# keya-dialog/LoCo-ASR

Hardware: AMD Instinct MI355X
Metric: audio frames/sec SpeechT5-base encoder, 30s×bs32 @1/2/4/8 GPU; embed L2 vs HF (higher is better)
Workload: dtype f16x3 (fp16 hi+lo operands, 3 MFMAs per product, fp32 accumulate); 1 GPU; SpeechT5-base speech encoder, synthetic 16 kHz 30 s clips, batch 32 per GPU (BASELINE.json configs[1]), random-init weights; batch_per_gpu=32, global_batch=32, frames_per_clip=1499, parallelism=dp1, collective=none

## Files before the change

### loco-asr_amd/csrc/attention_f16x3.hip

```cpp
#include <cstdlib>

#include "loco_kernels.h"

namespace loco {

typedef _Float16 h8 __attribute__((ext_vector_type(8)));
typedef float f32x2 __attribute__((ext_vector_type(2)));
typedef unsigned u32x4 __attribute__((ext_vector_type(4)));
typedef _Float16 h4 __attribute__((ext_vector_type(4)));

constexpr int AX_BQ = 128, AX_BK = 64;
constexpr int AX_PL = AX_BK * kHeadDim;
constexpr int AX_STG = 2 * AX_PL;

typedef __attribute__((address_space(1))) const void* ax_gptr_t;
typedef __attribute__((address_space(3))) void* ax_lptr_t;

#ifndef LOCO_ATTN_HACK
#define LOCO_ATTN_HACK 0
#endif
#define AX_MFMA(a, b, c) __builtin_amdgcn_mfma_f32_32x32x16_f16(a, b, c, 0, 0, 0)
#define AX_PIN() __builtin_amdgcn_sched_barrier(0)

#ifdef LOCO_ATTN_STAMPS
__device__ unsigned long long* g_attn_stamps = nullptr;
#define AX_STAMP(k_)                                                                                                     \
    {                                                                                                                    \
        unsigned long long t_;                                                                                           \
        __builtin_amdgcn_sched_barrier(0);                                                                               \
        asm volatile("s_memtime %0\n\ts_waitcnt lgkmcnt(0)" : "=s"(t_) :: "memory");                                     \
        __builtin_amdgcn_sched_barrier(0);                                                                               \
        seg[k_] += t_ - tlast;                                                                                           \
        tlast = t_;                                                                                                      \
    }
#else
#define AX_STAMP(k_) {}
#endif

__device__ __forceinline__ void ax_split_pair(const f32x2 pv, unsigned& hi, unsigned& lo) {
    asm("s_nop 0\n\tv_cvt_pk_f16_f32 %0, %1, %2" : "=v"(hi) : "v"(pv.x), "v"(pv.y));
    asm("v_fma_mixlo_f16 %0, %1, 1.0, -%2 op_sel_hi:[0,0,1]" : "=v"(lo) : "v"(pv.x), "v"(hi));
    asm("v_fma_mixhi_f16 %0, %1, 1.0, -%2 op_sel:[0,0,1] op_sel_hi:[0,0,1]" : "+v"(lo) : "v"(pv.y), "v"(hi));
}

#ifdef LOCO_ATTN_DEBUG
__device__ float* g_attn_dbg = nullptr;
#define AX_DBG(tile_, code_, S0_, S1_)                                                                                   \
    if (g_attn_dbg && (tile_) < 8) {                                                                                     \
        float* d_ = g_attn_dbg + (((long)blockIdx.x * 256 + tid) * 8 + (tile_)) * 8;                                     \
        unsigned mask_ = 0;                                                                                              \
        float smax_ = -INFINITY, smin_ = INFINITY;                                                                       \
        _Pragma("unroll") for (int e = 0; e < 16; ++e) {                                                                 \
            if (!(fabsf(S0_[e]) <= 3e38f) && S0_[e] != -INFINITY) mask_ |= 1u;                                           \
            if (!(fabsf(S1_[e]) <= 3e38f) && S1_[e] != -INFINITY) mask_ |= 1u;                                           \
            smax_ = fmaxf(smax_, fmaxf(S0_[e], S1_[e])); smin_ = fminf(smin_, fminf(S0_[e], S1_[e]));                    \
            if (!(fabsf(o0[e]) <= 3e38f) || !(fabsf(o1[e]) <= 3e38f)) mask_ |= 2u;                                       \
        }                                                                                                                \
        if (!(fabsf(l_run) <= 3e38f)) mask_ |= 4u;                                                                       \
        if (!(fabsf(alpha) <= 3e38f)) mask_ |= 8u;                                                                       \
        if (!(fabsf(dsh) <= 3e38f)) mask_ |= 16u;                                                                        \
        d_[0] = __uint_as_float(mask_ | ((code_) << 16)); d_[1] = m_run; d_[2] = alpha; d_[3] = dsh; d_[4] = l_run;      \
        d_[5] = smax_; d_[6] = smin_; d_[7] = o0[0];                                                                     \
    }
#else
#define AX_DBG(tile_, code_, S0_, S1_) {}
#endif

typedef __fp16 ax_tr4_t __attribute__((__vector_size__(4 * sizeof(__fp16))));
__device__ __forceinline__ h8 ax_join_tr(ax_tr4_t a, ax_tr4_t b) {
    const h4 x = __builtin_bit_cast(h4, a), y = __builtin_bit_cast(h4, b);
    return h8{x[0], x[1], x[2], x[3], y[0], y[1], y[2], y[3]};
}

template <bool OUT_SPLIT, bool TABLE, bool LONG_SEQ>
__global__ __launch_bounds__(256, 2) void attention_f16x3_kernel(const _Float16* __restrict__ qhi, const _Float16* __restrict__ qlo,
                                                                 const _Float16* __restrict__ khi, const _Float16* __restrict__ klo,
                                                                 const _Float16* __restrict__ vhi, const _Float16* __restrict__ vlo,
                                                                 float* qp, const int32_t* __restrict__ frames,
                                                                 _Float16* __restrict__ ctx_hi, _Float16* __restrict__ ctx_lo,
                                                                 float* __restrict__ ctx, int T, int nqb,
                                                                 const _Float16* __restrict__ pe_hi, const _Float16* __restrict__ pe_lo,
                                                                 float pe_scale) {
    __shared__ __attribute__((aligned(16))) _Float16 lds[4 * AX_STG];
    __shared__ __attribute__((aligned(16))) float bias_stage[4][32 * 17];

    int qblk, head, b;
    {
        const int nblk = gridDim.x;
        const int q8 = nblk >> 3, r8 = nblk & 7;
        const int xcd = blockIdx.x & 7, idx = blockIdx.x >> 3;
        const int w = (xcd < r8 ? xcd * (q8 + 1) : r8 * (q8 + 1) + (xcd - r8) * q8) + idx;
        qblk = w - (w / nqb) * nqb;
        const int rest = w / nqb;
        head = rest - (rest / kHeads) * kHeads;
        b = rest / kHeads;
    }
    const int tid = threadIdx.x, lane = tid & 63;
    const int wave = __builtin_amdgcn_readfirstlane(tid >> 6);
    const int r = lane & 31, h = lane >> 5;
    const int iw0 = qblk * AX_BQ + wave * 32;
    const int iq = iw0 + r;
    const int iqc = iq < T ? iq : T - 1;

    int nvalid = frames ? frames[b] : T;
    if (nvalid <= 0 || nvalid > T) nvalid = T;
    const int ntiles = (nvalid + AX_BK - 1) / AX_BK;
    constexpr float kLog2e = 1.4426950408889634f;

    h8 qh[4], ql[4];
    {
        const long qo = ((long)b * T + iqc) * kHidden + head * kHeadDim + 8 * h;
#pragma unroll
        for (int ks = 0; ks < 4; ++ks) {
            qh[ks] = *reinterpret_cast<const h8*>(qhi + qo + 16 * ks);
            ql[ks] = *reinterpret_cast<const h8*>(qlo + qo + 16 * ks);
        }
    }
    float* qprow = qp + (((long)b * kHeads + head) * T + iqc) * kRelN;

    const int drow = lane >> 3, dpos = lane & 7;
    const unsigned lds0 = (unsigned)(unsigned long)(ax_lptr_t)lds;
    unsigned kvc[2], vvc;
#pragma unroll
    for (int i = 0; i < 2; ++i) {
        const int swz = (((2 * wave + i) & 3) << 1) | ((drow >> 1) & 1);
        kvc[i] = 2u * (unsigned)(head * kHeadDim + 8 * (dpos ^ swz));
    }
    vvc = 2u * (unsigned)(head * kHeadDim + 8 * (dpos ^ (((drow >> 1) & 1) << 2)));
    const char* const kbase_h = reinterpret_cast<const char*>(khi + (long)b * T * kHidden);
    const char* const kbase_l = reinterpret_cast<const char*>(klo + (long)b * T * kHidden);
    const char* const vbase_h = reinterpret_cast<const char*>(vhi + (long)b * T * kHidden);
    const char* const vbase_l = reinterpret_cast<const char*>(vlo + (long)b * T * kHidden);
#define AX_DMA16(base_, voff_, ldsb_) \
    asm volatile("s_mov_b32 m0, %0\n\ts_nop 0\n\tglobal_load_lds_dwordx4 %1, %2" :: "s"(ldsb_), "v"(voff_), "s"(base_) : "memory")
#define AX_DMA_PIECE(pc_, tk_, tv_, kslot_, vslot_)                                                                          \
    {                                                                                                                        \
        const int i_ = ((pc_) >> 1) & 1, pl_ = (pc_) & 1;                                                                    \
        const bool isk_ = (pc_) < 4;                                                                                         \
        const int tt_ = isk_ ? (tk_) : (tv_);                                                                                \
        const int rmax_ = T - 1 - tt_ * AX_BK;           \
        int row_ = 8 * (2 * wave + i_) + drow;                                                                               \
        row_ = row_ < rmax_ ? row_ : rmax_;                                                                                  \
        const unsigned vo_ = (unsigned)row_ * (2u * kHidden) + (isk_ ? kvc[i_] : vvc);                                       \
        const unsigned d_ = lds0 + 2u * (unsigned)((isk_ ? (kslot_) : 2 + (vslot_)) * AX_STG + pl_ * AX_PL + 8 * (2 * wave + i_) * kHeadDim); \
        AX_DMA16((isk_ ? (pl_ ? kbase_l : kbase_h) : (pl_ ? vbase_l : vbase_h)) + (long)tt_ * (AX_BK * kHidden * 2), vo_, d_); \
    }

    int fo[4];
    {
        const int swz = (((r >> 3) & 3) << 1) | ((r >> 1) & 1);
#pragma unroll
        for (int y = 0; y < 4; ++y) fo[y] = r * kHeadDim + 8 * ((2 * y + h) ^ swz);
    }
#define AX_KF(kb_, st_, ks_, pl_) (*reinterpret_cast<const h8*>((kb_) + (pl_) * AX_PL + (st_) * 32 * kHeadDim + fo[ks_]))
    int vfo[2];
    {
        const int q = (lane >> 2) & 3, pp = lane & 3, g = (lane >> 4) & 1;
#pragma unroll
        for (int dt = 0; dt < 2; ++dt)
            vfo[dt] = (4 * h + q) * kHeadDim + 8 * ((4 * (dt ^ ((q >> 1) & 1))) + 2 * g + (pp >> 1)) + 4 * (pp & 1);
    }
    typedef __fp16 ax_tr4 __attribute__((__vector_size__(4 * sizeof(__fp16))));
    typedef __attribute__((address_space(3))) ax_tr4* ax_tr4_lptr;
#define AX_VTR(vb_, dt_, c_, u_, pl_) \
    __builtin_amdgcn_ds_read_tr16_b64_v4f16((ax_tr4_lptr)((vb_) + (pl_) * AX_PL + (16 * (c_) + 8 * (u_)) * kHeadDim + vfo[dt_]))
#define AX_VF(vb_, dt_, c_, pl_) ax_join_tr(AX_VTR(vb_, dt_, c_, 0, pl_), AX_VTR(vb_, dt_, c_, 1, pl_))

    f32x16 o0, o1;
#pragma unroll
    for (int e = 0; e < 16; ++e) { o0[e] = 0.f; o1[e] = 0.f; }
    float m_run = -INFINITY, l_run = 0.f;
    float alpha = 0.f, dsh = 0.f;

    float bandv[2][2][8];
#define AX_IS_BAND(tt_) (iw0 - ((tt_) * AX_BK + AX_BK - 1) < kRelMax - 1 && iw0 + 31 - (tt_) * AX_BK > -kRelMax)
#define AX_BAND_LOAD(tt_)                                                                                              \
    if (AX_IS_BAND(tt_)) {                                                                                             \
        const float* qpb = qp + ((long)b * kHeads + head) * T * kRelN;                                                 \
        const int lj = lane & 15, lq = lane >> 4;                                                                      \
        _Pragma("unroll") for (int st_ = 0; st_ < 2; ++st_)                                                            \
            _Pragma("unroll") for (int half = 0; half < 2; ++half) {                                                   \
                const int j = (tt_) * AX_BK + 32 * st_ + 16 * half + lj;                                               \
                _Pragma("unroll") for (int u = 0; u < 8; ++u) {                                                        \
                    const int i = iw0 + 4 * u + lq;                                                                    \
                    int rel = i - j;                                                                                   \
                    rel = rel < -kRelMax ? -kRelMax : (rel > kRelMax - 1 ? kRelMax - 1 : rel);                         \
                    bandv[st_][half][u] = qpb[(long)(i < T ? i : T - 1) * kRelN + rel + kRelMax];                      \
                }                                                                                                      \
            }                                                                                                          \
    }
#define AX_BAND_ADD(S_, st_)                                                                                           \
    _Pragma("unroll") for (int half = 0; half < 2; ++half) {                                                           \
        _Pragma("unroll") for (int u = 0; u < 8; ++u) sc[66 * u + band_wr] = bandv[st_][half][u];                      \
        __builtin_amdgcn_wave_barrier();                                                                               \
        _Pragma("unroll") for (int e8 = 0; e8 < 8; ++e8)                                                               \
            S_[8 * half + e8] += sc[band_rd + (e8 & 3) + 8 * (e8 >> 2)];                                               \
        __builtin_amdgcn_wave_barrier();                                                                               \
    }
#define AX_FINISH_TILE(S0_, S1_, tt_, mx_)                                                                             \
    {                                                                                                                  \
        const int j0 = (tt_) * AX_BK;                                                                                  \
        const int dmin = iw0 - (j0 + AX_BK - 1);                                                                       \
        const int dmax = iw0 + 31 - j0;                                                                                \
        float cb = 0.f;                                                                                                \
        bool redo = false;                                                                                             \
        if (dmin >= kRelMax - 1) {                                                                                     \
            cb = c_past;                                                                                               \
        } else if (dmax <= -kRelMax) {                                                                                 \
            cb = c_future;                                                                                             \
        } else {                                                                                                       \
            float* sc = bias_stage[wave];                                                                              \
            const int lj = lane & 15, lq = lane >> 4;                                                                  \
            const int band_wr = 16 * lq + (lq >> 1) + lj, band_rd = 16 * r + (r >> 1) + 4 * h;                         \
            AX_BAND_ADD(S0_, 0)                                                                                        \
            AX_BAND_ADD(S1_, 1)                                                                                        \
            redo = true;                                                                                               \
        }                                                                                                              \
        if (j0 + AX_BK > nvalid) {                                                                                     \
            _Pragma("unroll") for (int e = 0; e < 16; ++e) {                                                           \
                const int j = j0 + (e & 3) + 8 * (e >> 2) + 4 * h;                                                     \
                S0_[e] = j < nvalid ? S0_[e] : -INFINITY;                                                              \
                S1_[e] = j + 32 < nvalid ? S1_[e] : -INFINITY;                                                         \
            }                                                                                                          \
            redo = true;                                                                                               \
        }                                                                                                              \
        float mxv = (mx_);                                                                                             \
        if (redo) {                                                                                                    \
            mxv = S0_[0];                                                                                              \
            _Pragma("unroll") for (int e = 1; e < 16; ++e) mxv = fmaxf(mxv, S0_[e]);                                   \
            _Pragma("unroll") for (int e = 0; e < 16; ++e) mxv = fmaxf(mxv, S1_[e]);                                   \
        }                                                                                                              \
        {                                               \
            float ma_ = mxv, mb_ = mxv;                                                                                \
            asm volatile("s_nop 1\n\tv_permlane32_swap_b32 %0, %1\n\ts_nop 1" : "+v"(ma_), "+v"(mb_));                \
            mxv = fmaxf(ma_, mb_) + cb;                                                                                \
        }                                                                                                              \
        const float m_new = fmaxf(m_run, mxv);                                                                         \
        alpha = __builtin_amdgcn_exp2f((m_run - m_new) * kLog2e);                                                      \
        m_run = m_new;                                                                                                 \
        dsh = (cb - m_new) * kLog2e;                                                                                   \
    }

#ifdef LOCO_ATTN_STAMPS
    unsigned long long seg[6] = {0, 0, 0, 0, 0, 0}, tlast, tstart;
    asm volatile("s_memtime %0\n\ts_waitcnt lgkmcnt(0)" : "=s"(tstart) :: "memory");
    tlast = tstart;
#endif
#pragma unroll
    for (int pc = 0; pc < 8; ++pc) AX_DMA_PIECE(pc, 0, 0, 0, 0)
    float c_past, c_future;
    if (TABLE) {
        int bmin, bmax;
        {
            int lo = iw0 - (ntiles * AX_BK - 1), hi = iw0 + 31;
            lo = lo < -kRelMax ? -kRelMax : lo;
            hi = hi > kRelMax - 1 ? kRelMax - 1 : hi;
            bmin = (lo + kRelMax) >> 5;
            bmax = (hi + kRelMax) >> 5;
        }
        float cf = 0.f, cp = 0.f;
        unsigned pev[2];
#pragma unroll
        for (int i = 0; i < 2; ++i) {
            const int swz = (((2 * wave + i) & 3) << 1) | ((drow >> 1) & 1);
            pev[i] = (unsigned)(8 * (2 * wave + i) + drow) * (2u * kHeadDim) + 16u * (unsigned)(dpos ^ swz);
        }
        const unsigned bs0 = (unsigned)(unsigned long)(ax_lptr_t)&bias_stage[0][0];
        const unsigned pev1 = (unsigned)(8 * wave + drow) * (2u * kHeadDim) + 16u * (unsigned)(dpos ^ (((wave & 3) << 1) | ((drow >> 1) & 1)));
        constexpr int kBsPlane = 32 * kHeadDim;
#define AX_PE_DMA2(b0_, slot_)                                                                                                     \
    _Pragma("unroll") for (int pc_ = 0; pc_ < 4; ++pc_) {                                                                          \
        const int i_ = (pc_ >> 1) & 1, pl_ = pc_ & 1;                                                                              \
        const unsigned d_ = lds0 + 2u * (unsigned)((slot_) * AX_STG + pl_ * AX_PL + 8 * (2 * wave + i_) * kHeadDim);               \
        AX_DMA16(reinterpret_cast<const char*>(pl_ ? pe_lo : pe_hi) + (long)(b0_) * (32 * kHeadDim * 2), pev[i_], d_);             \
    }
#define AX_PE_DMA1(b0_)                                                                                                            \
    _Pragma("unroll") for (int pl_ = 0; pl_ < 2; ++pl_) {                                                                          \
        const unsigned d_ = bs0 + 2u * (unsigned)(pl_ * kBsPlane + 8 * wave * kHeadDim);                                           \
        AX_DMA16(reinterpret_cast<const char*>(pl_ ? pe_lo : pe_hi) + (long)(b0_) * (32 * kHeadDim * 2), pev1, d_);                \
    }
        constexpr int kBlocksPerRound = kRelN / 64;
        static_assert(2 * kBlocksPerRound * 32 == kRelN && sizeof(bias_stage) >= 2 * kBsPlane * sizeof(_Float16), "table rounds");
#define AX_PE_ROUND_DMA(rd_)                                                                      \
    AX_PE_DMA2(LOCO_ATTN_HACK == 1 ? 0 : kBlocksPerRound * (rd_), 1)                               \
    AX_PE_DMA2(LOCO_ATTN_HACK == 1 ? 0 : kBlocksPerRound * (rd_) + 2, 3)                           \
    AX_PE_DMA1(LOCO_ATTN_HACK == 1 ? 0 : kBlocksPerRound * (rd_) + 4)
        AX_PE_ROUND_DMA(0)
#pragma unroll
        for (int rd = 0; rd < 2; ++rd) {
            asm volatile("s_waitcnt vmcnt(0)" ::: "memory");
            __syncthreads();
            f32x16 acc[kBlocksPerRound];
#pragma unroll
            for (int bb = 0; bb < kBlocksPerRound; ++bb) {
                const _Float16* pb = bb == 4 ? reinterpret_cast<const _Float16*>(&bias_stage[0][0]) : lds + ((bb >> 1) ? 3 : 1) * AX_STG;
                const int plane = bb == 4 ? kBsPlane : AX_PL;
#pragma unroll
                for (int e = 0; e < 16; ++e) acc[bb][e] = 0.f;
                const int blk_ = kBlocksPerRound * rd + bb;
                if (blk_ < bmin || blk_ > bmax) continue;
#pragma unroll
                for (int ks = 0; ks < 4; ++ks) {
                    const h8 fh = *reinterpret_cast<const h8*>(pb + (bb & 1) * 32 * kHeadDim + fo[ks]);
                    const h8 fl = *reinterpret_cast<const h8*>(pb + plane + (bb & 1) * 32 * kHeadDim + fo[ks]);
                    acc[bb] = AX_MFMA(fl, qh[ks], acc[bb]);
                    acc[bb] = AX_MFMA(fh, ql[ks], acc[bb]);
                    acc[bb] = AX_MFMA(fh, qh[ks], acc[bb]);
                }
            }
            __syncthreads();
            if (rd == 0) {
                AX_PE_ROUND_DMA(1)
            } else {
                const int t1 = ntiles > 1 ? 1 : 0;
#pragma unroll
                for (int pc = 0; pc < 4; ++pc) AX_DMA_PIECE(pc, t1, 0, 1, 0)
            }
#pragma unroll
            for (int bb = 0; bb < kBlocksPerRound; ++bb) {
                const int blk = kBlocksPerRound * rd + bb;
#pragma unroll
                for (int e = 0; e < 16; ++e) acc[bb][e] *= pe_scale;
                if (blk == 0) cf = acc[bb][0];
                if (blk == kRelN / 32 - 1) cp = acc[bb][15];
                if (iq < T && blk >= bmin && blk <= bmax && (LOCO_ATTN_HACK != 2 || T < 0)) {
#pragma unroll
                    for (int g4 = 0; g4 < 4; ++g4)
                        *reinterpret_cast<float4*>(qprow + 32 * blk + 8 * g4 + 4 * h) =
                            make_float4(acc[bb][4 * g4], acc[bb][4 * g4 + 1], acc[bb][4 * g4 + 2], acc[bb][4 * g4 + 3]);
                }
            }
        }
#undef AX_PE_ROUND_DMA
#undef AX_PE_DMA2
#undef AX_PE_DMA1
        float cf2 = cf, cp2 = cp;
        asm volatile("s_nop 1\n\tv_permlane32_swap_b32 %0, %1\n\ts_nop 1" : "+v"(cf), "+v"(cf2));
        asm volatile("s_nop 1\n\tv_permlane32_swap_b32 %0, %1\n\ts_nop 1" : "+v"(cp2), "+v"(cp));
        c_future = cf;
        c_past = cp;
    } else {
        const int t1 = ntiles > 1 ? 1 : 0;
#pragma unroll
        for (int pc = 0; pc < 4; ++pc) AX_DMA_PIECE(pc, t1, 0, 1, 0)
        c_past = qprow[kRelN - 1];
        c_future = qprow[0];
    }
    asm volatile("s_waitcnt vmcnt(0)" ::: "memory");
    __syncthreads();

    f32x16 sa0, sa1, sb0, sb1;
    {
#pragma unroll
        for (int e = 0; e < 16; ++e) { sa0[e] = 0.f; sa1[e] = 0.f; }
        const _Float16* kb = lds;
#pragma unroll
        for (int ks = 0; ks < 4; ++ks) {
            const h8 kh0 = AX_KF(kb, 0, ks, 0), kl0 = AX_KF(kb, 0, ks, 1), kh1 = AX_KF(kb, 1, ks, 0), kl1 = AX_KF(kb, 1, ks, 1);
            sa0 = AX_MFMA(kl0, qh[ks], sa0); sa1 = AX_MFMA(kl1, qh[ks], sa1);
            sa0 = AX_MFMA(kh0, ql[ks], sa0); sa1 = AX_MFMA(kh1, ql[ks], sa1);
            sa0 = AX_MFMA(kh0, qh[ks], sa0); sa1 = AX_MFMA(kh1, qh[ks], sa1);
        }
        float mx = sa0[0];
#pragma unroll
        for (int e = 1; e < 16; ++e) mx = fmaxf(mx, sa0[e]);
#pragma unroll
        for (int e = 0; e < 16; ++e) mx = fmaxf(mx, sa1[e]);
        AX_BAND_LOAD(0)
        AX_FINISH_TILE(sa0, sa1, 0, mx)
    }
    __syncthreads();
    AX_STAMP(5)

#define AX_ITER(t_, SC0, SC1, SN0, SN1)                                                                                \
    {                                                                                                                  \
        const int tq = (t_);                                                                                           \
        const int tkn = tq + 2 < ntiles ? tq + 2 : ntiles - 1, tvn = tq + 1 < ntiles ? tq + 1 : ntiles - 1;             \
        if (tq + 1 < ntiles) { AX_BAND_LOAD(tq + 1) }                                                                  \
        const _Float16* kb = lds + ((tq + 1) & 1) * AX_STG;                                                            \
        const _Float16* vb = lds + (2 + (tq & 1)) * AX_STG;                                                            \
        h8 kf[2][4];                                                                 \
        kf[0][0] = AX_KF(kb, 0, 0, 0); kf[0][1] = AX_KF(kb, 0, 0, 1);                                                  \
        kf[0][2] = AX_KF(kb, 1, 0, 0); kf[0][3] = AX_KF(kb, 1, 0, 1);                                                  \
        const f32x2 al2 = {alpha, alpha}, k2 = {kLog2e, kLog2e}, d2 = {dsh, dsh};                                      \
        f32x2 ps2 = {0.f, 0.f};                                                                                        \
           \
        if (!LONG_SEQ || __builtin_amdgcn_ballot_w64(alpha != 1.0f) != 0) {                                            \
            _Pragma("unroll") for (int e = 0; e < 16; e += 2) {                                                        \
                f32x2 a_ = {o0[e], o0[e + 1]}, c_ = {o1[e], o1[e + 1]};                                                \
                a_ *= al2; c_ *= al2;                                                                                  \
                o0[e] = a_.x; o0[e + 1] = a_.y; o1[e] = c_.x; o1[e + 1] = c_.y;                                        \
            }                                                                                                          \
        }                                                                                                              \
        _Pragma("unroll") for (int e = 0; e < 16; ++e) { SN0[e] = 0.f; SN1[e] = 0.f; }                                 \
        u32x4 ph0[2], pl0[2], ph1[2], pl1[2];                                                                          \
        AX_PIN();                                                                                                      \
        AX_STAMP(0)                                                                                                    \
                                                                                                     \
        _Pragma("unroll") for (int ks = 0; ks < 4; ++ks) {                                                             \
            if (ks + 1 < 4) {                                                                                          \
                kf[(ks + 1) & 1][0] = AX_KF(kb, 0, ks + 1, 0); kf[(ks + 1) & 1][1] = AX_KF(kb, 0, ks + 1, 1);          \
                kf[(ks + 1) & 1][2] = AX_KF(kb, 1, ks + 1, 0); kf[(ks + 1) & 1][3] = AX_KF(kb, 1, ks + 1, 1);          \
            }                                                                                                          \
            _Pragma("unroll") for (int m = 0; m < 6; ++m) {                                                            \
                const int st = m & 1, wh = m >> 1;                                                                     \
                const h8 a_ = kf[ks & 1][2 * st + (wh == 0 ? 1 : 0)];                                                  \
                const h8 b_ = wh == 1 ? ql[ks] : qh[ks];                                                               \
                if (st == 0) SN0 = AX_MFMA(a_, b_, SN0); else SN1 = AX_MFMA(a_, b_, SN1);                              \
                const int n = 6 * ks + m, q_ = n / 3;                                                                  \
                if (n % 3 == 0) {                                                                                      \
                    const int e0 = 2 * q_;                                                                             \
                    const f32x2 sx = {SC0[e0], SC0[e0 + 1]};                                                           \
                    const f32x2 ax = __builtin_elementwise_fma(sx, k2, d2);                                            \
                    const f32x2 pv = {__builtin_amdgcn_exp2f(ax.x), __builtin_amdgcn_exp2f(ax.y)};                     \
                    ps2 += pv;                                                                                         \
                    asm volatile("" : "+v"(ps2));                                                                      \
                    unsigned hi_, lo_;                                                                                 \
                    ax_split_pair(pv, hi_, lo_);                                                                       \
                    ph0[q_ >> 2][q_ & 3] = hi_; pl0[q_ >> 2][q_ & 3] = lo_;                                            \
                } else if (n % 3 == 1) {                                                                               \
                    const int e0 = 2 * q_;                                                                             \
                    const f32x2 sx = {SC1[e0], SC1[e0 + 1]};                                                           \
                    const f32x2 ax = __builtin_elementwise_fma(sx, k2, d2);                                            \
                    SC1[e0] = __builtin_amdgcn_exp2f(ax.x); SC1[e0 + 1] = __builtin_amdgcn_exp2f(ax.y);                \
                }                                                                                                      \
                if (n % 3 == 1 && (LOCO_ATTN_HACK != 3 || ((n / 3) & 1) == 0)) {  \
                    AX_PIN();                                                                                          \
                    AX_DMA_PIECE(n / 3, tkn, tvn, tq & 1, (tq + 1) & 1)                                                \
                }                                                                                                      \
                AX_PIN();                                                                                              \
            }                                                                                                          \
        }                                                                                                              \
        AX_STAMP(1)                                                                                                    \
                             \
        h8 vf[2][2];                                                                             \
        vf[0][0] = AX_VF(vb, 0, 0, 0); vf[0][1] = AX_VF(vb, 0, 0, 1);                                                  \
        float mxr = -INFINITY;                                                                                         \
        _Pragma("unroll") for (int g = 0; g < 8; ++g) {                                                                \
            const int st = g >> 2, s2 = (g >> 1) & 1, dt = g & 1;                                                      \
            if (g + 1 < 8) {                                                                                           \
                const int c1 = (g + 1) >> 1, dt1 = (g + 1) & 1;                                                        \
                vf[(g + 1) & 1][0] = AX_VF(vb, dt1, c1, 0); vf[(g + 1) & 1][1] = AX_VF(vb, dt1, c1, 1);                \
            }                                                                                                          \
            const h8 vh = vf[g & 1][0], vl = vf[g & 1][1];                                                             \
            const h8 ph = __builtin_bit_cast(h8, st == 0 ? ph0[s2] : ph1[s2]);                                         \
            const h8 pl = __builtin_bit_cast(h8, st == 0 ? pl0[s2] : pl1[s2]);                                         \
            _Pragma("unroll") for (int m = 0; m < 3; ++m) {                                                            \
                const h8 a_ = m == 0 ? vl : vh;                                                                        \
                const h8 b_ = m == 1 ? pl : ph;                                                                        \
                if (dt == 0) o0 = AX_MFMA(a_, b_, o0); else o1 = AX_MFMA(a_, b_, o1);                                  \
                const int n = 3 * g + m;                                                                               \
                if (n < 8) {                          \
                    const f32x2 pv = {SC1[2 * n], SC1[2 * n + 1]};                                                     \
                    ps2 += pv;                                                                                         \
                    asm volatile("" : "+v"(ps2));                                                                      \
                    unsigned hi_, lo_;                                                                                 \
                    ax_split_pair(pv, hi_, lo_);                                                                       \
                    ph1[n >> 2][n & 3] = hi_; pl1[n >> 2][n & 3] = lo_;                                                \
                } else if (n >= 12 && n < 20) {              \
                    const int e0 = 4 * (n - 12);                                                                       \
                    if (e0 < 16) mxr = fmaxf(fmaxf(fmaxf(mxr, SN0[e0]), fmaxf(SN0[e0 + 1], SN0[e0 + 2])), SN0[e0 + 3]); \
                    else mxr = fmaxf(fmaxf(fmaxf(mxr, SN1[e0 - 16]), fmaxf(SN1[e0 - 15], SN1[e0 - 14])), SN1[e0 - 13]); \
                    asm volatile("" : "+v"(mxr));                                                                      \
                }                                                                                                      \
                AX_PIN();                                                                                              \
            }                                                                                                          \
        }                                                                                                              \
        l_run = l_run * alpha + (ps2.x + ps2.y);                                                                       \
        AX_STAMP(2)                                                                                                    \
        if (tq + 1 < ntiles) { AX_FINISH_TILE(SN0, SN1, tq + 1, mxr) }                                                 \
        AX_DBG(tq, 1u, SN0, SN1)                                                                                       \
        AX_STAMP(3)                                                                                                    \
        asm volatile("s_waitcnt vmcnt(0)" ::: "memory");                                                               \
        __syncthreads();                                                                                               \
        AX_STAMP(4)                                                                                                    \
    }

    for (int t = 0; t < ntiles; t += 2) {
        AX_ITER(t, sa0, sa1, sb0, sb1)
        if (t + 1 >= ntiles) break;
        AX_ITER(t + 1, sb0, sb1, sa0, sa1)
    }
#undef AX_ITER
#undef AX_FINISH_TILE
#undef AX_BAND_LOAD
#undef AX_BAND_ADD
#undef AX_IS_BAND
#undef AX_DMA_PIECE
#undef AX_DMA16
#undef AX_KF
#undef AX_VF
#undef AX_VTR

#ifdef LOCO_ATTN_STAMPS
    if (g_attn_stamps && tid == 0) {
        unsigned long long* o_ = g_attn_stamps + 8l * blockIdx.x;
        for (int k_ = 0; k_ < 6; ++k_) o_[k_] = seg[k_];
        o_[6] = (unsigned long long)ntiles;
        o_[7] = tlast - tstart;
    }
#endif
    const float l_tot = l_run + __shfl_xor(l_run, 32, 64);
    const float inv = 1.0f / l_tot;
    if (iq < T) {
        const long obase = ((long)b * T + iq) * kHidden + head * kHeadDim + 4 * h;
#pragma unroll
        for (int g4 = 0; g4 < 4; ++g4) {
            float a[4], c[4];
#pragma unroll
            for (int e = 0; e < 4; ++e) {
                a[e] = o0[4 * g4 + e] * inv;
                c[e] = o1[4 * g4 + e] * inv;
            }
            if (OUT_SPLIT) {
                typedef unsigned u32x2 __attribute__((ext_vector_type(2)));
                unsigned h0, l0, h1, l1;
                split_f16_2pairs(a[0], a[1], a[2], a[3], h0, l0, h1, l1);
                *reinterpret_cast<u32x2*>(ctx_hi + obase + 8 * g4) = u32x2{h0, h1};
                *reinterpret_cast<u32x2*>(ctx_lo + obase + 8 * g4) = u32x2{l0, l1};
                split_f16_2pairs(c[0], c[1], c[2], c[3], h0, l0, h1, l1);
                *reinterpret_cast<u32x2*>(ctx_hi + obase + 32 + 8 * g4) = u32x2{h0, h1};
                *reinterpret_cast<u32x2*>(ctx_lo + obase + 32 + 8 * g4) = u32x2{l0, l1};
            } else {
                *reinterpret_cast<float4*>(ctx + obase + 8 * g4) = make_float4(a[0], a[1], a[2], a[3]);
                *reinterpret_cast<float4*>(ctx + obase + 32 + 8 * g4) = make_float4(c[0], c[1], c[2], c[3]);
            }
        }
    }
}

static int read_attn_long_knob() {
    const char* v = getenv("LOCO_ATTN_LONG");
    return v ? (atoi(v) != 0) : -1;
}
static int& attn_long_knob() {
    static int k = read_attn_long_knob();
    return k;
}
void reload_attention_knobs() { attn_long_knob() = read_attn_long_knob(); }

hipError_t launch_attention_f16x3(const _Float16* qhi, const _Float16* qlo, const _Float16* khi, const _Float16* klo,
                                  const _Float16* vhi, const _Float16* vlo, const float* qp, const int32_t* frames,
                                  _Float16* ctx_hi, _Float16* ctx_lo, float* ctx, int B, int T, hipStream_t s,
                                  const _Float16* pe_hi, const _Float16* pe_lo, float pe_scale) {
    if (B <= 0 || T <= 0 || B > 65535) return hipErrorInvalidValue;
    const int nqb = (T + AX_BQ - 1) / AX_BQ;
    const long nblk = (long)nqb * kHeads * B;
    if (nblk > 0x7fffffffL) return hipErrorInvalidValue;
    dim3 grid((unsigned)nblk);
    float* qpw = const_cast<float*>(qp);
    if ((pe_hi == nullptr) != (pe_lo == nullptr)) return hipErrorInvalidValue;
    const int forced = attn_long_knob();
    const bool long_seq = forced < 0 ? T >= 4096 : forced != 0;
#define AX_LAUNCH1(SPLIT_, TABLE_, LONG_)                                                                                              \
    hipLaunchKernelGGL((attention_f16x3_kernel<SPLIT_, TABLE_, LONG_>), grid, dim3(256), 0, s, qhi, qlo, khi, klo, vhi, vlo, qpw, frames, ctx_hi, \
                       ctx_lo, ctx, T, nqb, pe_hi, pe_lo, pe_scale)
#define AX_LAUNCH(SPLIT_, TABLE_)                    \
    {                                                \
        if (long_seq) AX_LAUNCH1(SPLIT_, TABLE_, true); \
        else AX_LAUNCH1(SPLIT_, TABLE_, false);      \
    }
    if (ctx_hi && pe_hi) AX_LAUNCH(true, true)
    else if (ctx_hi) AX_LAUNCH(true, false)
    else if (pe_hi) AX_LAUNCH(false, true)
    else AX_LAUNCH(false, false)
#undef AX_LAUNCH
#undef AX_LAUNCH1
    return hipGetLastError();
}

}

#ifdef LOCO_ATTN_DEBUG
extern "C" int loco_debug_set_attn_dbg(void* buf) {
    return (int)hipMemcpyToSymbol(HIP_SYMBOL(loco::g_attn_dbg), &buf, sizeof(buf));
}
#endif
#ifdef LOCO_ATTN_STAMPS
extern "C" int loco_debug_set_attn_stamps(void* buf) {
    return (int)hipMemcpyToSymbol(HIP_SYMBOL(loco::g_attn_stamps), &buf, sizeof(buf));
}
#endif
```

Baseline: 949,100 frames/s.

## Transpose positional-score MFMA and repack split context stores with permlane swaps

The relative-position score MFMAs now take swapped operands, so each lane holds a column of results. Those results are written straight to the per-row qp table with scalar strided stores and a partial-tile guard, and c_past/c_future are read back from qprow after the barrier instead of being exchanged with permlane swaps. The split fp16 hi/lo context output now uses permlane32 swaps to assemble 16-byte vector stores in place of 8-byte stores. The intent is wider output stores and a simpler edge-value path. The cost is many scalar strided global stores for the qp table, and new dependencies on iqc, r and the row mapping being correct.

```diff
diff --git a/loco-asr_amd/csrc/attention_f16x3.hip b/loco-asr_amd/csrc/attention_f16x3.hip
--- a/loco-asr_amd/csrc/attention_f16x3.hip
+++ b/loco-asr_amd/csrc/attention_f16x3.hip
@@ -258,7 +258,8 @@
             bmin = (lo + kRelMax) >> 5;
             bmax = (hi + kRelMax) >> 5;
         }
-        float cf = 0.f, cp = 0.f;
+        float* const qpst = qp + (((long)b * kHeads + head) * T + iw0) * kRelN + (4 * h * kRelN + r);
+        const int nrow = T - iw0 - 4 * h;
         unsigned pev[2];
 #pragma unroll
         for (int i = 0; i < 2; ++i) {
@@ -303,9 +304,9 @@
                 for (int ks = 0; ks < 4; ++ks) {
                     const h8 fh = *reinterpret_cast<const h8*>(pb + (bb & 1) * 32 * kHeadDim + fo[ks]);
                     const h8 fl = *reinterpret_cast<const h8*>(pb + plane + (bb & 1) * 32 * kHeadDim + fo[ks]);
-                    acc[bb] = AX_MFMA(fl, qh[ks], acc[bb]);
-                    acc[bb] = AX_MFMA(fh, ql[ks], acc[bb]);
-                    acc[bb] = AX_MFMA(fh, qh[ks], acc[bb]);
+                    acc[bb] = AX_MFMA(qh[ks], fl, acc[bb]);
+                    acc[bb] = AX_MFMA(ql[ks], fh, acc[bb]);
+                    acc[bb] = AX_MFMA(qh[ks], fh, acc[bb]);
                 }
             }
             __syncthreads();
@@ -321,24 +322,21 @@
                 const int blk = kBlocksPerRound * rd + bb;
 #pragma unroll
                 for (int e = 0; e < 16; ++e) acc[bb][e] *= pe_scale;
-                if (blk == 0) cf = acc[bb][0];
-                if (blk == kRelN / 32 - 1) cp = acc[bb][15];
-                if (iq < T && blk >= bmin && blk <= bmax && (LOCO_ATTN_HACK != 2 || T < 0)) {
-#pragma unroll
-                    for (int g4 = 0; g4 < 4; ++g4)
-                        *reinterpret_cast<float4*>(qprow + 32 * blk + 8 * g4 + 4 * h) =
-                            make_float4(acc[bb][4 * g4], acc[bb][4 * g4 + 1], acc[bb][4 * g4 + 2], acc[bb][4 * g4 + 3]);
+                if (blk >= bmin && blk <= bmax && (LOCO_ATTN_HACK != 2 || T < 0)) {
+                    if (iw0 + 32 <= T) {
+#pragma unroll
+                        for (int e = 0; e < 16; ++e) qpst[((e & 3) + 8 * (e >> 2)) * kRelN + 32 * blk] = acc[bb][e];
+                    } else {
+#pragma unroll
+                        for (int e = 0; e < 16; ++e)
+                            if ((e & 3) + 8 * (e >> 2) < nrow) qpst[((e & 3) + 8 * (e >> 2)) * kRelN + 32 * blk] = acc[bb][e];
+                    }
                 }
             }
         }
 #undef AX_PE_ROUND_DMA
 #undef AX_PE_DMA2
 #undef AX_PE_DMA1
-        float cf2 = cf, cp2 = cp;
-        asm volatile("s_nop 1\n\tv_permlane32_swap_b32 %0, %1\n\ts_nop 1" : "+v"(cf), "+v"(cf2));
-        asm volatile("s_nop 1\n\tv_permlane32_swap_b32 %0, %1\n\ts_nop 1" : "+v"(cp2), "+v"(cp));
-        c_future = cf;
-        c_past = cp;
     } else {
         const int t1 = ntiles > 1 ? 1 : 0;
 #pragma unroll
@@ -348,6 +346,10 @@
     }
     asm volatile("s_waitcnt vmcnt(0)" ::: "memory");
     __syncthreads();
+    if (TABLE) {
+        c_past = qprow[kRelN - 1];
+        c_future = qprow[0];
+    }
 
     f32x16 sa0, sa1, sb0, sb1;
     {
@@ -502,7 +504,31 @@
 #endif
     const float l_tot = l_run + __shfl_xor(l_run, 32, 64);
     const float inv = 1.0f / l_tot;
-    if (iq < T) {
+    if (OUT_SPLIT) {
+        const long obase = ((long)b * T + iqc) * kHidden + head * kHeadDim + 8 * h;
+#pragma unroll
+        for (int dt = 0; dt < 2; ++dt) {
+#pragma unroll
+            for (int pr = 0; pr < 2; ++pr) {
+                unsigned ph_[2][2], pl_[2][2];
+#pragma unroll
+                for (int k = 0; k < 2; ++k) {
+                    const int e0 = 4 * (2 * pr + k);
+                    if (dt == 0) split_f16_2pairs(o0[e0] * inv, o0[e0 + 1] * inv, o0[e0 + 2] * inv, o0[e0 + 3] * inv, ph_[k][0], pl_[k][0], ph_[k][1], pl_[k][1]);
+                    else split_f16_2pairs(o1[e0] * inv, o1[e0 + 1] * inv, o1[e0 + 2] * inv, o1[e0 + 3] * inv, ph_[k][0], pl_[k][0], ph_[k][1], pl_[k][1]);
+                }
+#pragma unroll
+                for (int w = 0; w < 2; ++w) {
+                    asm volatile("s_nop 1\n\tv_permlane32_swap_b32 %0, %1\n\ts_nop 1" : "+v"(ph_[0][w]), "+v"(ph_[1][w]));
+                    asm volatile("s_nop 1\n\tv_permlane32_swap_b32 %0, %1\n\ts_nop 1" : "+v"(pl_[0][w]), "+v"(pl_[1][w]));
+                }
+                if (iq < T) {
+                    *reinterpret_cast<u32x4*>(ctx_hi + obase + 32 * dt + 16 * pr) = u32x4{ph_[0][0], ph_[0][1], ph_[1][0], ph_[1][1]};
+                    *reinterpret_cast<u32x4*>(ctx_lo + obase + 32 * dt + 16 * pr) = u32x4{pl_[0][0], pl_[0][1], pl_[1][0], pl_[1][1]};
+                }
+            }
+        }
+    } else if (iq < T) {
         const long obase = ((long)b * T + iq) * kHidden + head * kHeadDim + 4 * h;
 #pragma unroll
         for (int g4 = 0; g4 < 4; ++g4) {
@@ -512,19 +538,8 @@
                 a[e] = o0[4 * g4 + e] * inv;
                 c[e] = o1[4 * g4 + e] * inv;
             }
-            if (OUT_SPLIT) {
-                typedef unsigned u32x2 __attribute__((ext_vector_type(2)));
-                unsigned h0, l0, h1, l1;
-                split_f16_2pairs(a[0], a[1], a[2], a[3], h0, l0, h1, l1);
-                *reinterpret_cast<u32x2*>(ctx_hi + obase + 8 * g4) = u32x2{h0, h1};
-                *reinterpret_cast<u32x2*>(ctx_lo + obase + 8 * g4) = u32x2{l0, l1};
-                split_f16_2pairs(c[0], c[1], c[2], c[3], h0, l0, h1, l1);
-                *reinterpret_cast<u32x2*>(ctx_hi + obase + 32 + 8 * g4) = u32x2{h0, h1};
-                *reinterpret_cast<u32x2*>(ctx_lo + obase + 32 + 8 * g4) = u32x2{l0, l1};
-            } else {
-                *reinterpret_cast<float4*>(ctx + obase + 8 * g4) = make_float4(a[0], a[1], a[2], a[3]);
-                *reinterpret_cast<float4*>(ctx + obase + 32 + 8 * g4) = make_float4(c[0], c[1], c[2], c[3]);
-            }
+            *reinterpret_cast<float4*>(ctx + obase + 8 * g4) = make_float4(a[0], a[1], a[2], a[3]);
+            *reinterpret_cast<float4*>(ctx + obase + 32 + 8 * g4) = make_float4(c[0], c[1], c[2], c[3]);
         }
     }
 }
```

New measurement: 953,900 frames/s (median of 6 runs). About the same (+0.5%).
